# yumingj/C2-Matching

Hardware: AMD Instinct MI355X
Metric: LR-Ref image pairs/sec (160x160 LR, 500x500 Ref, 4x SR) (higher is better)
Workload: dtype f32

## Files before the change

### c2-matching_amd/c2m_amd/_lib.py

```python
import ctypes
import os

import torch

_HERE = os.path.dirname(os.path.abspath(__file__))
LIB_PATH = os.environ.get("C2M_LIB") or os.path.join(os.path.dirname(_HERE), "csrc", "libc2m_hip.so")
ABI_VERSION = 4

_vp, _i, _sz = ctypes.c_void_p, ctypes.c_int, ctypes.c_size_t
_lib = None


class ConvSrc(ctypes.Structure):
    _fields_ = [("ptr", _vp), ("C", _i), ("pix_pitch", _i), ("row_pitch", _i), ("img_pitch", ctypes.c_longlong)]


class Conv3x3Desc(ctypes.Structure):
    _fields_ = [("B", _i), ("H", _i), ("W", _i), ("Cin", _i), ("Cout", _i), ("nsrc", _i), ("src", ConvSrc * 2),
                ("wr", _vp), ("bias", _vp), ("act", _i), ("slope", ctypes.c_float), ("out_mode", _i), ("out", _vp),
                ("out_pix_pitch", _i), ("out_row_pitch", _i), ("out_img_pitch", ctypes.c_longlong), ("res1", _vp),
                ("res2", _vp), ("mask_out", _vp), ("flow", _vp), ("fh", _i), ("fw", _i), ("scale", _i), ("n_off", _i),
                ("abs_sum", _vp), ("algo", _i), ("cout_offset", _i), ("cout_total", _i),
                ("out2", _vp), ("out2_row_pitch", _i), ("out2_plane_pitch", ctypes.c_longlong),
                ("out2_img_pitch", ctypes.c_longlong), ("range_flag", _vp), ("io_flags", ctypes.c_int)]
# ... 8 lines not shown
    L.c2m_status_string.restype = ctypes.c_char_p
    L.c2m_status_string.argtypes = [_i]
    L.c2m_last_hip_error.restype = ctypes.c_char_p
    L.c2m_device_arch.argtypes = [ctypes.c_char_p, _i]
    L.c2m_profile_enable.argtypes = [_i]
    L.c2m_profile_collect.argtypes = [ctypes.POINTER(ctypes.c_float), ctypes.POINTER(_i), _i, ctypes.POINTER(_i)]
    L.c2m_feature_normalize_f32.argtypes = [_vp, _vp, _i, _i, _i, _vp]
    L.c2m_feature_match_workspace_bytes.restype = _sz
    L.c2m_feature_match_workspace_bytes.argtypes = [_i] * 5
    L.c2m_feature_match_workspace_bytes_c.restype = _sz
    L.c2m_feature_match_workspace_bytes_c.argtypes = [_i] * 6
    L.c2m_feature_match_skip_table.argtypes = [_i] * 5 + [ctypes.POINTER(ctypes.c_size_t), ctypes.POINTER(ctypes.c_int)]
    L.c2m_feature_match_index_f32.argtypes = [_vp, _vp, _vp] + [_i] * 12 + [_vp, _vp, _vp, _sz]
    L.c2m_feature_match_index_pre_f32.argtypes = [_vp, _vp, _vp] + [_i] * 12 + [_vp, _vp, _vp, _sz, _vp, _vp]
    L.c2m_feature_match_index_pre_f32.restype = _i
    L.c2m_feature_normalize_ss_f32.argtypes = [_vp, _vp, _i, _i, _i, _vp, _vp]
    L.c2m_feature_normalize_ss_f32.restype = _i
    L.c2m_feature_match_set_filter.argtypes = [_i]
    L.c2m_conv3x3_set_head_stores.argtypes = [_i]
    L.c2m_feature_match_filter_tables.argtypes = [_i] * 5 + [ctypes.POINTER(ctypes.c_size_t)] * 3 + [ctypes.POINTER(ctypes.c_int)]
    L.c2m_build_pre_offsets_f32.argtypes = [_vp, _vp, _i, _i, _i, _vp, _vp, _vp]
    for name in ("c2m_dcn_v2_forward_workspace_bytes",):
        getattr(L, name).restype = _sz
        getattr(L, name).argtypes = [_i] * 8
    L.c2m_dcn_v2_backward_workspace_bytes.restype = _sz
    L.c2m_dcn_v2_backward_workspace_bytes.argtypes = [_i] * 14
    L.c2m_dcn_v2_forward_f32.argtypes = [_vp] * 6 + [_i] * 14 + [_vp, _vp, _sz]
    L.c2m_dcn_v2_forward_bf16mma_f32.argtypes = [_vp] * 6 + [_i] * 14 + [_vp, _vp, _sz]
    L.c2m_dcn_v2_backward_f32.argtypes = [_vp] * 7 + [_i] * 14 + [_vp] * 5 + [_vp, _sz]
    L.c2m_dcn_fuse_offsets_f32.argtypes = [_vp, _vp, _vp, _i, _i, _i, _i, _i, _vp, _vp, _vp]
# ... 82 lines not shown
```

### c2-matching_amd/c2m_amd/ops.py

```python
import torch

from . import _lib


def _dev_f32(t, name):
    if not isinstance(t, torch.Tensor) or not t.is_cuda:
        raise _lib.C2MError(f"{name} must be a tensor on the GPU (the HIP path has no CPU fallback)")
    if t.dtype != torch.float32:
        raise _lib.C2MError(f"{name} must be float32, got {t.dtype}")
    return t if t.is_contiguous() else t.contiguous()


def _stream():
    return torch.cuda.current_stream().cuda_stream


def _pair(v):
    return (int(v), int(v)) if isinstance(v, int) else (int(v[0]), int(v[1]))


class NormalizedFeatures(torch.Tensor):

    @staticmethod
    def wrap(t, ss):
# ... 54 lines not shown
                                                         idx.data_ptr(), val.data_ptr(), ws.data_ptr(), nbytes,
                                                         ss_i.data_ptr() if ss_i is not None else None,
                                                         ss_r.data_ptr() if ss_r is not None else None),
                       "c2m_feature_match_index_pre_f32")
        mfma = (not force_generic) and p == 3 and si == 1 and sr == 1 and C in (64, 128, 256)
        if return_skip or _corr_diag.enabled:
            table = _skip_table(ws, (B, Hq, Wq, Hr, Wr)) if mfma else None
            if _corr_diag.enabled:
                _corr_diag.table = table
                _corr_diag.filter = _filter_tables(ws, (B, Hq, Wq, Hr, Wr), Hqp * Wqp) if mfma else None
            if return_skip:
                if table is None:
                    raise _lib.C2MError("return_skip: the duplicate-row table exists only on the MFMA kernel's path "
                                        "(patch 3, strides 1, C in 64/128/256, force_generic=False)")
                return idx, val, table
    return idx, val


class _CorrDiag:
    enabled = False
    table = None
    filter = None


_corr_diag = _CorrDiag()


class record_corr_skip_table:
    def __enter__(self):
        _corr_diag.enabled, _corr_diag.table = True, None
# ... 1181 lines not shown
```

### c2-matching_amd/csrc/corr_argmax.hip

```cpp
#include <stdlib.h>

#include "c2m_common.h"
#include "corr_filter.h"

namespace c2m {


__global__ void __launch_bounds__(256) feature_normalize_kernel(const float* __restrict__ x, int C, int HW,
                                                                 float* __restrict__ out, float* __restrict__ ss_out) {
  const int p = blockIdx.x * 256 + threadIdx.x;
  if (p >= HW) return;
  const float* xb = x + (size_t)blockIdx.y * C * HW + p;
  float* ob = out + (size_t)blockIdx.y * C * HW + p;
  float ss = 0.0f;
  for (int c = 0; c < C; ++c) {
    const float v = xb[(size_t)c * HW];
    ss = fmaf(v, v, ss);
  }
  const float nrm = sqrtf(ss);
  const float den = nrm > 1e-12f ? nrm : 1e-12f;
  float s2 = 0.0f;
  for (int c = 0; c < C; ++c) {
    const float o = xb[(size_t)c * HW] / den;
    ob[(size_t)c * HW] = o;
// ... 13 lines not shown
#pragma unroll
  for (int c = 0; c < C; ++c) v[c] = xb[(size_t)c * HW];
  float ss = 0.0f;
#pragma unroll
  for (int c = 0; c < C; ++c) ss = fmaf(v[c], v[c], ss);
  const float nrm = sqrtf(ss);
  const float den = nrm > 1e-12f ? nrm : 1e-12f;
  float s2 = 0.0f;
#pragma unroll
  for (int c = 0; c < C; ++c) {
    const float o = v[c] / den;
    ob[(size_t)c * HW] = o;
    s2 = fmaf(o, o, s2);
  }
  if (ss_out) ss_out[(size_t)blockIdx.y * HW + p] = s2;
}

__global__ void __launch_bounds__(256) pixel_sumsq_kernel(const float* __restrict__ x, int C, int HW,
                                                           float* __restrict__ ss) {
  const int p = blockIdx.x * 256 + threadIdx.x;
  if (p >= HW) return;
  const float* xb = x + (size_t)blockIdx.y * C * HW + p;
  float a = 0.0f;
  for (int c = 0; c < C; ++c) {
    const float v = xb[(size_t)c * HW];
    a = fmaf(v, v, a);
  }
  ss[(size_t)blockIdx.y * HW + p] = a;
}

// ... 392 lines not shown
    (void)hipMemsetAsync(row_eq, 0, sizeof(int) * (size_t)B * nxt * Hr, st);
  }
  hipLaunchKernelGGL(ref_row_run_kernel, dim3(ceil_div(B * nxt, 64)), dim3(64), 0, st, row_eq, Hr, B * nxt, skip);
  const int* need = nullptr;
  if (fws) {
    if (int rc = c2m::corrf::launch(st, fin, fref, B, C, Hq, Wq, Hr, Wr, inv, qden_buf, qden ? 1 : 0, skip, wsbase, *fws, max_idx,
                                    max_val))
      return rc;
    need = reinterpret_cast<const int*>(wsbase + fws->flags);
  }
  ProfileScope prof(C2M_KERNEL_CORR_MFMA, st);
  hipLaunchKernelGGL(kern, grid, dim3(NTHR), lds, st, fin, fref, Hq, Wq, Hr, Wr, tiles_y, tiles_x, inv ? inv : fin,
                     qden ? qden : fin, inv ? 1 : 0, qden ? 1 : 0, skip, need, max_idx, max_val);
  return check_launch();
}
}

namespace {
thread_local int g_filter_mode = -1;
}

extern "C" int c2m_feature_match_set_filter(int mode) {
  if (mode < -1 || mode > 1) return C2M_ERR_INVALID_ARG;
  g_filter_mode = mode;
  return C2M_OK;
}

extern "C" int c2m_feature_match_filter_tables(int B, int Hq, int Wq, int Hr, int Wr, size_t* cnt_offset, size_t* cand_offset,
                                               size_t* flags_offset, int* slots) {
  if (B <= 0 || Hq <= 0 || Wq <= 0 || Hr <= 0 || Wr <= 0 || !cnt_offset || !cand_offset || !flags_offset || !slots)
// ... 12 lines not shown
}

static int filter_channels(int C) { return (C == 64 || C == 128 || C == 256) ? C : 0; }

extern "C" size_t c2m_feature_match_workspace_bytes_c(int B, int C, int Hq, int Wq, int Hr, int Wr) {
  if (B <= 0 || C <= 0 || Hq <= 0 || Wq <= 0 || Hr <= 0 || Wr <= 0) return 0;
  return corr_ws(B, Hq, Wq, Hr, Wr, filter_channels(C)).total;
}

extern "C" int c2m_feature_match_skip_table(int B, int Hq, int Wq, int Hr, int Wr, size_t* byte_offset, int* x_tiles) {
  if (B <= 0 || Hq <= 0 || Wq <= 0 || Hr <= 0 || Wr <= 0 || !byte_offset || !x_tiles) return C2M_ERR_INVALID_ARG;
  const CorrWs ws = corr_ws(B, Hq, Wq, Hr, Wr);
  *byte_offset = ws.skip;
  *x_tiles = ws.nxt;
  return C2M_OK;
}

extern "C" int c2m_feature_match_index_f32(c2m_stream_t stream, const float* feat_in, const float* feat_ref, int B,
                                           int C, int Hq, int Wq, int Hr, int Wr, int patch, int in_stride,
                                           int ref_stride, int is_norm, int norm_input, int force_generic,
                                           int64_t* max_idx, float* max_val, void* workspace,
                                           size_t workspace_bytes) {
  return c2m_feature_match_index_pre_f32(stream, feat_in, feat_ref, B, C, Hq, Wq, Hr, Wr, patch, in_stride, ref_stride, is_norm,
                                         norm_input, force_generic, max_idx, max_val, workspace, workspace_bytes, nullptr, nullptr);
}

extern "C" int c2m_feature_match_index_pre_f32(c2m_stream_t stream, const float* feat_in, const float* feat_ref, int B,
                                               int C, int Hq, int Wq, int Hr, int Wr, int patch, int in_stride,
                                               int ref_stride, int is_norm, int norm_input, int force_generic,
                                               int64_t* max_idx, float* max_val, void* workspace,
// ... 11 lines not shown
  float* qden = reinterpret_cast<float*>(wsb + ws.qden);

  const int Hqp = (Hq - patch) / in_stride + 1, Wqp = (Wq - patch) / in_stride + 1;
  const int Hrp = (Hr - patch) / ref_stride + 1, Wrp = (Wr - patch) / ref_stride + 1;
  int rc;
  if (is_norm) {
    if (!ss_ref_pre)
      hipLaunchKernelGGL(pixel_sumsq_kernel, dim3(ceil_div(Hr * Wr, 256), B), dim3(256), 0, st, feat_ref, C, Hr * Wr,
                         ss_ref);
    hipLaunchKernelGGL(patch_norm_kernel, dim3(ceil_div(Hrp * Wrp, 256), B), dim3(256), 0, st, ss_ref_pre ? ss_ref_pre : ss_ref, Hr, Wr, patch,
                       ref_stride, Hrp, Wrp, 1, inv);
    if ((rc = check_launch()) != C2M_OK) return rc;
  }
  const bool fast = !force_generic && patch == 3 && in_stride == 1 && ref_stride == 1 &&
                    (C == 64 || C == 128 || C == 256);
  static const int filter_env = [] {
    const char* e = getenv("C2M_CORR_FILTER");
    return (e && e[0] == '0') ? 0 : 1;
  }();
  const int filter_on = g_filter_mode < 0 ? filter_env : g_filter_mode;
  const bool use_filter = fast && filter_on && is_norm && c2m::corrf::shapes_ok(B, C, Hq, Wq, Hr, Wr);
  if (norm_input || use_filter) {
    if (!ss_in_pre)
      hipLaunchKernelGGL(pixel_sumsq_kernel, dim3(ceil_div(Hq * Wq, 256), B), dim3(256), 0, st, feat_in, C, Hq * Wq,
                         ss_in);
    hipLaunchKernelGGL(patch_norm_kernel, dim3(ceil_div(Hqp * Wqp, 256), B), dim3(256), 0, st, ss_in_pre ? ss_in_pre : ss_in, Hq, Wq, patch,
                       in_stride, Hqp, Wqp, 0, qden);
    if ((rc = check_launch()) != C2M_OK) return rc;
  }
  const float* invp = is_norm ? inv : nullptr;
  const float* qdp = norm_input ? qden : nullptr;

  if (fast) {
    int* row_eq = reinterpret_cast<int*>(wsb + ws.row_eq);
    int2* skip = reinterpret_cast<int2*>(wsb + ws.skip);
    const c2m::corrf::Ws* fwsp = use_filter ? &ws.f : nullptr;
    static const int dedup = [] {
      const char* e = getenv("C2M_CORR_DEDUP");
      return (e && e[0] == '0') ? 0 : 1;
    }();
    if (C == 256)
      return launch_corr_mfma<256>(st, feat_in, feat_ref, B, Hq, Wq, Hr, Wr, invp, qdp, row_eq, skip, dedup, max_idx,
                                   max_val, fwsp, wsb, qden);
    if (C == 128)
      return launch_corr_mfma<128>(st, feat_in, feat_ref, B, Hq, Wq, Hr, Wr, invp, qdp, row_eq, skip, dedup, max_idx,
                                   max_val, fwsp, wsb, qden);
    return launch_corr_mfma<64>(st, feat_in, feat_ref, B, Hq, Wq, Hr, Wr, invp, qdp, row_eq, skip, dedup, max_idx,
                                max_val, fwsp, wsb, qden);
  }
  const size_t lds = sizeof(float) * (size_t)patch * patch * C;
  if (lds > 60 * 1024) return C2M_ERR_UNSUPPORTED;
  ProfileScope prof(C2M_KERNEL_CORR_GENERIC, st);
  hipLaunchKernelGGL(corr_argmax_generic_kernel, dim3(Hqp * Wqp, B), dim3(256), lds, st, feat_in, feat_ref, C, Hq, Wq,
                     Hr, Wr, patch, in_stride, ref_stride, Wqp, Hrp, Wrp, invp, qdp, max_idx, max_val);
  return check_launch();
// ... 17 lines not shown
```

### c2-matching_amd/csrc/corr_filter.h

```cpp
#pragma once
#include <hip/hip_runtime.h>
#include <stddef.h>
#include <stdint.h>

namespace c2m {
namespace corrf {

constexpr int WP = 28;
constexpr int KSLOT = 8;
constexpr int SCAN_ITEMS = 8192;
constexpr int CMAX = 256;

struct Ws {
  size_t qn, rn;
  size_t qpl;
  size_t rimg;
  size_t sb;
  size_t band;
  size_t eq;
  size_t cnt;
  size_t cand;
  size_t flags;
  size_t keys;
  size_t items;
// ... 27 lines not shown
  w.total = o;
  return w;
}

inline bool shapes_ok(int B, int C, int Hq, int Wq, int Hr, int Wr) {
  if (!(C == 64 || C == 128 || C == 256)) return false;
  if (Hr - 2 > 1024 || (Wr - 2 + WP - 1) / WP > 64) return false;
  const size_t lim = (size_t)1 << 31;
  const size_t nxt = (size_t)(Wr - 2 + WP - 1) / WP;
  return (size_t)Hq * Wq * C * 4 < lim && (size_t)Hr * Wr * C * 4 < lim && nxt * Hr * C * 128 < lim;
}

int launch(hipStream_t st, const float* fin, const float* fref, int B, int C, int Hq, int Wq, int Hr, int Wr, const float* inv,
           const float* qden, int norm_input, int2* skip, char* wsbase, const Ws& ws, int64_t* max_idx, float* max_val);

}
}
```

### c2-matching_amd/csrc/corr_filter.hip

```cpp
#include "corr_filter.h"

#include <stdlib.h>

#include "c2m_common.h"

namespace c2m {
namespace corrf {

constexpr int TQ = 16, TPQ = TQ - 2, WT = 32, NWAVE = 8, NTHR = NWAVE * 64, QPIX = TQ * TQ, SLAB = QPIX * WT, NIT = TPQ;
constexpr float BAND_ALPHA = 8.4e-5f, BAND_BETA = 1.0e-6f, INV_CAP = 2.0f;
constexpr float PIECE_SCALE = 16384.0f;
constexpr float SCORE_UNSCALE = 3.725290298461914e-9f;
constexpr float F16_MIN_NORMAL = 6.103515625e-5f;
constexpr int SCAN_FLAG = 0x40000000;
constexpr int SCAN_CAP = SCAN_ITEMS;
constexpr int SCAN_CHUNKS = 32, SCAN_STRIPES = 64;

typedef _Float16 f16x8 __attribute__((ext_vector_type(8)));


__global__ void __launch_bounds__(256) to_nhwc_kernel(const float* __restrict__ in, int C, int HW, float* __restrict__ out) {
  __shared__ float tile[64][65];
  const int b = blockIdx.z, c0 = blockIdx.y * 64, p0 = blockIdx.x * 64;
  const int tx = threadIdx.x & 63, ty = threadIdx.x >> 6;
// ... 48 lines not shown
  }
  if (bad) flags[0] = 1;
}

__device__ __forceinline__ void split2(float x, _Float16& h0, _Float16& h1, bool& bad) {
  const float xs = x * PIECE_SCALE;
  const float ax = __builtin_fabsf(xs);
  bad |= !(ax < 65520.0f);
  const _Float16 a = ax < F16_MIN_NORMAL ? (_Float16)0.0f : (_Float16)xs;
  const float r = xs - (float)a;
  const _Float16 c = __builtin_fabsf(r) < F16_MIN_NORMAL ? (_Float16)0.0f : (_Float16)r;
  h0 = a;
  h1 = c;
}

__device__ __forceinline__ void split8(const float* __restrict__ src, f16x8& p0, f16x8& p1, bool& bad) {
  const f32x4 a = *reinterpret_cast<const f32x4*>(src), c = *reinterpret_cast<const f32x4*>(src + 4);
#pragma unroll
  for (int e = 0; e < 4; ++e) {
    _Float16 h0, h1;
    split2(a[e], h0, h1, bad);
    p0[e] = h0; p1[e] = h1;
    split2(c[e], h0, h1, bad);
    p0[4 + e] = h0; p1[4 + e] = h1;
  }
}

__global__ void __launch_bounds__(256) split_query_kernel(const float* __restrict__ qn, int C, int HW, long long n8,
                                                           _Float16* __restrict__ qpl, int* __restrict__ flags) {
  const long long e = (long long)blockIdx.x * 256 + threadIdx.x;
  if (e >= n8) return;
  const int c8 = (int)(e % (C / 8));
  const long long gp = e / (C / 8);
  const long long b = gp / HW, p = gp - b * HW;
  f16x8 p0, p1;
  bool bad = false;
  split8(qn + (size_t)gp * C + c8 * 8, p0, p1, bad);
  _Float16* o = qpl + ((size_t)(b * 2) * HW + p) * C + c8 * 8;
  *reinterpret_cast<f16x8*>(o) = p0;
  *reinterpret_cast<f16x8*>(o + (size_t)HW * C) = p1;
// ... 32 lines not shown
    const u32x4 v = *me;
    if (x > 0) {
      const u32x4 o = *(me - C / 4);
      okl = v[0] == o[0] && v[1] == o[1] && v[2] == o[2] && v[3] == o[3];
    }
    if (y > 0) {
      const u32x4 o = *(me - (size_t)Wr * (C / 4));
      oku = v[0] == o[0] && v[1] == o[1] && v[2] == o[2] && v[3] == o[3];
    }
  }
  okl = __all(okl) && x > 0;
  oku = __all(oku) && y > 0;
  if (l == 0) {
    eq[gp] = okl ? 1 : 0;
    eq[npix + gp] = oku ? 1 : 0;
  }
}

__global__ void __launch_bounds__(256) cand_scale_kernel(const float* __restrict__ inv, const unsigned char* __restrict__ eq,
                                                          long long npix, int Hr, int Wr, int Hrp, int Wrp,
                                                          float* __restrict__ sc, int* __restrict__ flags, int* __restrict__ maxcol) {
  const int n0 = blockIdx.x * 256 + threadIdx.x, b = blockIdx.y;
  const bool in = n0 < Hrp * Wrp;
  const int n = in ? n0 : 0;
  const int ry = n / Wrp, rx = n - ry * Wrp;
  const unsigned char* el = eq + (size_t)b * Hr * Wr + (size_t)ry * Wr + rx;
  const unsigned char* eu = el + npix;
  bool dl = true, du = true;
#pragma unroll
  for (int i = 0; i < 3; ++i)
// ... 402 lines not shown
template <int C>
static int launch_filter_c(hipStream_t st, const _Float16* qpl, const _Float16* rimg, int B, int Hq, int Wq, int Hr, int Wr,
                           const float* sc, const float* band, const int2* skip, int* cnt, int* cand) {
  const int tiles_y = ceil_div(Hq - 2, TPQ), tiles_x = ceil_div(Wq - 2, TPQ);
  const size_t lds = sizeof(float) * (size_t)(3 * SLAB) + 2 * (size_t)C * 128;
  static const int pf = [] { const char* e = getenv("C2M_CORR_PF"); return (e && e[0] == '2') ? 2 : 1; }();
  static unsigned long long lds_set[2] = {0, 0};
  auto kern = pf == 1 ? &corr_filter_kernel<C, 1> : &corr_filter_kernel<C, 2>;
  if (int rc = ensure_dynamic_lds(reinterpret_cast<const void*>(kern), lds, lds_set[pf - 1])) return rc;
  ProfileScope prof(C2M_KERNEL_CORR_FILTER, st);
  hipLaunchKernelGGL(kern, dim3(B * tiles_y * tiles_x), dim3(NTHR), lds, st, qpl, rimg, Hq, Wq, Hr, Wr, tiles_y, tiles_x, sc, band,
                     skip, cnt, cand);
  return check_launch();
}

int launch(hipStream_t st, const float* fin, const float* fref, int B, int C, int Hq, int Wq, int Hr, int Wr, const float* inv,
           const float* qden, int norm_input, int2* skip, char* wsbase, const Ws& ws, int64_t* max_idx, float* max_val) {
  float* qn = reinterpret_cast<float*>(wsbase + ws.qn);
  float* rn = reinterpret_cast<float*>(wsbase + ws.rn);
  _Float16* qpl = reinterpret_cast<_Float16*>(wsbase + ws.qpl);
  _Float16* rimg = reinterpret_cast<_Float16*>(wsbase + ws.rimg);
  float* sc = reinterpret_cast<float*>(wsbase + ws.sb);
  float* band = reinterpret_cast<float*>(wsbase + ws.band);
  unsigned char* eq = reinterpret_cast<unsigned char*>(wsbase + ws.eq);
  int* cnt = reinterpret_cast<int*>(wsbase + ws.cnt);
  int* cand = reinterpret_cast<int*>(wsbase + ws.cand);
  int* flags = reinterpret_cast<int*>(wsbase + ws.flags);
  unsigned long long* keys = reinterpret_cast<unsigned long long*>(wsbase + ws.keys);
  ScanItem* items = reinterpret_cast<ScanItem*>(wsbase + ws.items);
  const int HWq = Hq * Wq, HWr = Hr * Wr, Hqp = Hq - 2, Wqp = Wq - 2, Hrp = Hr - 2, Wrp = Wr - 2;
  const int nxt = ceil_div(Wrp, WP);
  const long long nqp = (long long)B * Hqp * Wqp, npix_r = (long long)B * HWr;

  int* maxcol = reinterpret_cast<int*>(wsbase + ws.maxcol);
  static const int dead_tiles = [] { const char* e = getenv("C2M_CORR_DEAD_TILES"); return e ? atoi(e) : 1; }();
  (void)hipMemsetAsync(flags, 0, 32, st);
  (void)hipMemsetAsync(maxcol, 0, sizeof(int) * (size_t)B, st);
  hipLaunchKernelGGL(to_nhwc_split_kernel, dim3(ceil_div(HWq, 64), C / 64, B), dim3(256), 0, st, fin, C, HWq, qn, qpl, flags);
  hipLaunchKernelGGL(to_nhwc_kernel, dim3(ceil_div(HWr, 64), C / 64, B), dim3(256), 0, st, fref, C, HWr, rn);
  hipLaunchKernelGGL(split_ref_image_kernel, dim3(Hr, nxt, B), dim3(256), 0, st, rn, C, Hr, Wr, nxt, rimg, flags);
  hipLaunchKernelGGL(pixel_eq_kernel, dim3((unsigned)((npix_r + 3) / 4)), dim3(256), 0, st, rn, C, Hr, Wr, npix_r, eq);
  hipLaunchKernelGGL(cand_scale_kernel, dim3(ceil_div(Hrp * Wrp, 256), B), dim3(256), 0, st, inv, eq, npix_r, Hr, Wr, Hrp, Wrp, sc,
                     flags, maxcol);
  if (dead_tiles) hipLaunchKernelGGL(dead_tiles_kernel, dim3(ceil_div(B * nxt, 64)), dim3(64), 0, st, maxcol, nxt, B * nxt, Hr, skip);
  hipLaunchKernelGGL(band_kernel, dim3((unsigned)((nqp + 255) / 256)), dim3(256), 0, st, qden, nqp, band);
  int rc = check_launch();
  if (rc != C2M_OK) return rc;
  if (C == 256) rc = launch_filter_c<256>(st, qpl, rimg, B, Hq, Wq, Hr, Wr, sc, band, skip, cnt, cand);
  else if (C == 128) rc = launch_filter_c<128>(st, qpl, rimg, B, Hq, Wq, Hr, Wr, sc, band, skip, cnt, cand);
  else rc = launch_filter_c<64>(st, qpl, rimg, B, Hq, Wq, Hr, Wr, sc, band, skip, cnt, cand);
  if (rc != C2M_OK) return rc;
  {
    ProfileScope prof(C2M_KERNEL_CORR_RESOLVE, st);
    hipLaunchKernelGGL(corr_resolve_kernel, dim3((unsigned)((nqp + 27) / 28)), dim3(256), 0, st, qn, rn, C, Hq, Wq, Hr, Wr, inv, qden,
                       norm_input, cnt, cand, nqp, keys, items, flags, max_idx, max_val);
    hipLaunchKernelGGL(corr_scan_kernel, dim3(SCAN_CHUNKS, SCAN_STRIPES), dim3(256), 0, st, qn, rn, C, Hq, Wq, Hr, Wr, inv, items, flags,
                       keys);
    hipLaunchKernelGGL(corr_scan_finish_kernel, dim3(8), dim3(256), 0, st, items, flags, keys, qden, norm_input, max_idx, max_val);
  }
  return check_launch();
}

}
}
```

### c2-matching_amd/mmsr/models/archs/corres_generation_arch.py

```python
import logging

import torch
import torch.nn as nn

from c2m_amd import ops as _ops
from mmsr.models.archs.vgg_arch import VGGFeatureExtractor

logger = logging.getLogger('base')


class PreOffsets(dict):

    _SCALE = {'relu3_1': 1, 'relu2_1': 2, 'relu1_1': 4}

    def __init__(self, max_idx, h=None, w=None):
        super().__init__()
        if isinstance(max_idx, torch.Tensor):
            dict.__setitem__(self, 'max_idx', max_idx)
        else:
            for k, v in dict(max_idx).items():
                dict.__setitem__(self, k, v)
            if not dict.__contains__(self, 'max_idx'):
                raise TypeError("PreOffsets needs the arg-max index map (a tensor, or a mapping with key 'max_idx')")
        mi = dict.__getitem__(self, 'max_idx')
# ... 34 lines not shown
        super(CorrespondenceGenerationArch, self).__init__()
        self.patch_size = patch_size
        self.stride = stride
        self.vgg_layer_list = vgg_layer_list
        self.vgg = VGGFeatureExtractor(layer_name_list=vgg_layer_list, vgg_type=vgg_type)
        self.vgg.grouped8_taps = ('relu1_1',)
        self.vgg.fast_conv = True

    def index_to_flow(self, max_idx):
        h, w = max_idx.shape
        (flow,) = _ops.build_pre_offsets(max_idx[None].contiguous(), h + 2, w + 2, scales=(1,))
        return flow[:, 0]

    @torch.no_grad()
    def match(self, dense_features):
        feat_in = _ops.feature_normalize(dense_features['dense_features1'].float(), with_sumsq=True)
        feat_ref = _ops.feature_normalize(dense_features['dense_features2'].float(), with_sumsq=True)
        return _ops.feature_match_index_batched(feat_in, feat_ref, self.patch_size, self.stride, self.stride,
                                                is_norm=True, norm_input=True)

    def forward(self, dense_features, img_ref_hr):
        if self.patch_size != 3 or self.stride != 1:
            raise NotImplementedError('pre-offset generation is defined for patch_size=3, stride=1')
        h, w = dense_features['dense_features1'].shape[2:]
        max_idx, _ = self.match(dense_features)
        pre_offset = PreOffsets(max_idx, h, w)
        img_ref_feat = self.vgg(img_ref_hr)
        return pre_offset, img_ref_feat
```

### include/c2m_hip.h

```cpp
#ifndef C2M_HIP_H
#define C2M_HIP_H

#include <stddef.h>
#include <stdint.h>

#ifdef __cplusplus
extern "C" {
#endif

typedef void* c2m_stream_t;

typedef enum c2m_status {
  C2M_OK = 0,
  C2M_ERR_INVALID_ARG = 1,
  C2M_ERR_UNSUPPORTED = 2,
  C2M_ERR_WORKSPACE = 3,
  C2M_ERR_LAUNCH = 4,
  C2M_ERR_NO_DEVICE = 5
} c2m_status;

int c2m_abi_version(void);
const char* c2m_status_string(int status);
const char* c2m_last_hip_error(void);
int c2m_device_arch(char* buf, int buflen);
// ... 20 lines not shown
int c2m_feature_match_set_filter(int mode);

int c2m_conv3x3_set_head_stores(int mode);

int c2m_feature_match_filter_tables(int B, int Hq, int Wq, int Hr, int Wr, size_t* cnt_offset, size_t* cand_offset,
                                    size_t* flags_offset, int* slots);

int c2m_feature_match_index_f32(c2m_stream_t stream, const float* feat_in, const float* feat_ref, int B, int C,
                                int Hq, int Wq, int Hr, int Wr, int patch, int in_stride, int ref_stride,
                                int is_norm, int norm_input, int force_generic, int64_t* max_idx, float* max_val,
                                void* workspace, size_t workspace_bytes);
int c2m_feature_match_index_pre_f32(c2m_stream_t stream, const float* feat_in, const float* feat_ref, int B, int C,
                                    int Hq, int Wq, int Hr, int Wr, int patch, int in_stride, int ref_stride,
                                    int is_norm, int norm_input, int force_generic, int64_t* max_idx, float* max_val,
                                    void* workspace, size_t workspace_bytes, const float* ss_in_pre, const float* ss_ref_pre);

int c2m_build_pre_offsets_f32(c2m_stream_t stream, const int64_t* max_idx, int B, int h, int w, float* off3,
                              float* off2, float* off1);

size_t c2m_dcn_v2_forward_workspace_bytes(int B, int C, int H, int W, int Co, int kh, int kw, int dg);
int c2m_dcn_v2_forward_f32(c2m_stream_t stream, const float* input, const float* weight, const float* bias,
                           const float* offset, const float* mask, int B, int C, int H, int W, int Co, int kh, int kw,
                           int sh, int sw, int ph, int pw, int dh, int dw, int dg, float* output, void* workspace,
                           size_t workspace_bytes);

int c2m_dcn_v2_forward_bf16mma_f32(c2m_stream_t stream, const float* input, const float* weight, const float* bias,
                                   const float* offset, const float* mask, int B, int C, int H, int W, int Co, int kh,
                                   int kw, int sh, int sw, int ph, int pw, int dh, int dw, int dg, float* output,
                                   void* workspace, size_t workspace_bytes);

// ... 120 lines not shown
```

Measured before the change: 119.9.

## Fuse feature normalization into correlation filter prep from raw features

Adds a raw-input entry point for the correlation-argmax path. Instead of normalizing features to NCHW and then transposing them to NHWC for the filter, one kernel normalizes, writes NHWC, and emits the fp16 split planes. A single kernel also builds the split ref image and the row/pixel equality tables. The NCHW normalized tensors are only produced, via conditional kernels, when the filter flags a fallback to the MFMA kernel. This cuts several passes over feature memory and launches, but it adds a new code path, an extra scratch allocation per call, and 256-float register arrays per thread.

```diff
diff --git a/c2-matching_amd/c2m_amd/_lib.py b/c2-matching_amd/c2m_amd/_lib.py
--- a/c2-matching_amd/c2m_amd/_lib.py
+++ b/c2-matching_amd/c2m_amd/_lib.py
@@ -46,6 +46,8 @@
     L.c2m_feature_match_index_f32.argtypes = [_vp, _vp, _vp] + [_i] * 12 + [_vp, _vp, _vp, _sz]
     L.c2m_feature_match_index_pre_f32.argtypes = [_vp, _vp, _vp] + [_i] * 12 + [_vp, _vp, _vp, _sz, _vp, _vp]
     L.c2m_feature_match_index_pre_f32.restype = _i
+    L.c2m_feature_match_index_raw_f32.argtypes = [_vp, _vp, _vp] + [_i] * 12 + [_vp, _vp, _vp, _sz, _vp, _vp]
+    L.c2m_feature_match_index_raw_f32.restype = _i
     L.c2m_feature_normalize_ss_f32.argtypes = [_vp, _vp, _i, _i, _i, _vp, _vp]
     L.c2m_feature_normalize_ss_f32.restype = _i
     L.c2m_feature_match_set_filter.argtypes = [_i]
diff --git a/c2-matching_amd/c2m_amd/ops.py b/c2-matching_amd/c2m_amd/ops.py
--- a/c2-matching_amd/c2m_amd/ops.py
+++ b/c2-matching_amd/c2m_amd/ops.py
@@ -92,6 +92,37 @@
                     raise _lib.C2MError("return_skip: the duplicate-row table exists only on the MFMA kernel's path "
                                         "(patch 3, strides 1, C in 64/128/256, force_generic=False)")
                 return idx, val, table
+    return idx, val
+
+
+def feature_match_index_raw(raw_in, raw_ref, patch_size=3, stride=1, norm_input=True):
+    ok = all(isinstance(t, torch.Tensor) and t.is_cuda and t.dtype == torch.float32 and t.dim() == 4 for t in (raw_in, raw_ref))
+    if not ok or raw_in.shape[:2] != raw_ref.shape[:2] or raw_in.device != raw_ref.device:
+        return None
+    fi, fr = raw_in.contiguous(), raw_ref.contiguous()
+    B, C, Hq, Wq = fi.shape
+    Hr, Wr = fr.shape[2:]
+    p, s = int(patch_size), int(stride)
+    if min(Hq, Wq, Hr, Wr) < p or p != 3 or s != 1 or C not in (64, 128, 256):
+        return None
+    Hqp, Wqp = (Hq - p) // s + 1, (Wq - p) // s + 1
+    L = _lib.lib()
+    with torch.cuda.device(fi.device):
+        nbytes = L.c2m_feature_match_workspace_bytes_c(B, C, Hq, Wq, Hr, Wr)
+        ws = torch.empty(nbytes, dtype=torch.uint8, device=fi.device)
+        idx = torch.empty((B, Hqp, Wqp), dtype=torch.int64, device=fi.device)
+        val = torch.empty((B, Hqp, Wqp), dtype=torch.float32, device=fi.device)
+        ni, nr = torch.empty_like(fi), torch.empty_like(fr)
+        with _apply_switch("filter"):
+            rc = L.c2m_feature_match_index_raw_f32(_stream(), fi.data_ptr(), fr.data_ptr(), B, C, Hq, Wq, Hr, Wr, p, s, s, 1,
+                                                   int(bool(norm_input)), 0, idx.data_ptr(), val.data_ptr(), ws.data_ptr(), nbytes,
+                                                   ni.data_ptr(), nr.data_ptr())
+        if rc == 2:
+            return None
+        _lib.check(rc, "c2m_feature_match_index_raw_f32")
+        if _corr_diag.enabled:
+            _corr_diag.table = _skip_table(ws, (B, Hq, Wq, Hr, Wr))
+            _corr_diag.filter = _filter_tables(ws, (B, Hq, Wq, Hr, Wr), Hqp * Wqp)
     return idx, val
 
 
diff --git a/c2-matching_amd/csrc/corr_argmax.hip b/c2-matching_amd/csrc/corr_argmax.hip
--- a/c2-matching_amd/csrc/corr_argmax.hip
+++ b/c2-matching_amd/csrc/corr_argmax.hip
@@ -51,6 +51,26 @@
     s2 = fmaf(o, o, s2);
   }
   if (ss_out) ss_out[(size_t)blockIdx.y * HW + p] = s2;
+}
+
+template <int C>
+__global__ void __launch_bounds__(256, 1) feature_normalize_if_kernel(const float* __restrict__ x, int HW, float* __restrict__ out,
+                                                                       const int* __restrict__ need) {
+  if (*need == 0) return;
+  const int p = blockIdx.x * 256 + threadIdx.x;
+  if (p >= HW) return;
+  const float* xb = x + (size_t)blockIdx.y * C * HW + p;
+  float* ob = out + (size_t)blockIdx.y * C * HW + p;
+  float v[C];
+#pragma unroll
+  for (int c = 0; c < C; ++c) v[c] = xb[(size_t)c * HW];
+  float ss = 0.0f;
+#pragma unroll
+  for (int c = 0; c < C; ++c) ss = fmaf(v[c], v[c], ss);
+  const float nrm = sqrtf(ss);
+  const float den = nrm > 1e-12f ? nrm : 1e-12f;
+#pragma unroll
+  for (int c = 0; c < C; ++c) ob[(size_t)c * HW] = v[c] / den;
 }
 
 __global__ void __launch_bounds__(256) pixel_sumsq_kernel(const float* __restrict__ x, int C, int HW,
@@ -473,6 +493,34 @@
                      qden ? qden : fin, inv ? 1 : 0, qden ? 1 : 0, skip, need, max_idx, max_val);
   return check_launch();
 }
+
+template <int C>
+int launch_corr_raw(hipStream_t st, const float* raw_in, const float* raw_ref, int B, int Hq, int Wq, int Hr, int Wr, float* ss_in,
+                    float* ss_ref, float* inv, float* qden, int norm_input, int* row_eq, int2* skip, int dedup, int64_t* max_idx,
+                    float* max_val, const c2m::corrf::Ws& fws, char* wsbase, float* norm_in, float* norm_ref) {
+  using namespace c2m::corr;
+  const int tiles_y = ceil_div(Hq - 2, TPQ), tiles_x = ceil_div(Wq - 2, TPQ);
+  const int Hqp = Hq - 2, Wqp = Wq - 2, Hrp = Hr - 2, Wrp = Wr - 2, nxt = ceil_div(Wrp, WP);
+  const size_t lds = sizeof(float) * (size_t)(3 * SLAB + 2 * C * WT);
+  static unsigned long long lds_set[2] = {0, 0};
+  const bool dma16 = (Wr % 4 == 0) && (reinterpret_cast<uintptr_t>(norm_ref) % 16 == 0);
+  auto kern = dma16 ? &corr_argmax_mfma_kernel<C, true> : &corr_argmax_mfma_kernel<C, false>;
+  if (int rc = ensure_dynamic_lds(reinterpret_cast<const void*>(kern), lds, lds_set[dma16])) return rc;
+  if (int rc = c2m::corrf::prepare_raw(st, raw_in, raw_ref, B, C, Hq, Wq, Hr, Wr, ss_in, ss_ref, row_eq, wsbase, fws)) return rc;
+  if (!dedup) (void)hipMemsetAsync(row_eq, 0, sizeof(int) * (size_t)B * nxt * Hr, st);
+  hipLaunchKernelGGL(patch_norm_kernel, dim3(ceil_div(Hrp * Wrp, 256), B), dim3(256), 0, st, ss_ref, Hr, Wr, 3, 1, Hrp, Wrp, 1, inv);
+  hipLaunchKernelGGL(patch_norm_kernel, dim3(ceil_div(Hqp * Wqp, 256), B), dim3(256), 0, st, ss_in, Hq, Wq, 3, 1, Hqp, Wqp, 0, qden);
+  hipLaunchKernelGGL(ref_row_run_kernel, dim3(ceil_div(B * nxt, 64)), dim3(64), 0, st, row_eq, Hr, B * nxt, skip);
+  if (int rc = check_launch()) return rc;
+  if (int rc = c2m::corrf::sweep(st, B, C, Hq, Wq, Hr, Wr, inv, qden, norm_input, skip, wsbase, fws, max_idx, max_val)) return rc;
+  const int* need = reinterpret_cast<const int*>(wsbase + fws.flags);
+  hipLaunchKernelGGL(feature_normalize_if_kernel<C>, dim3(ceil_div(Hq * Wq, 256), B), dim3(256), 0, st, raw_in, Hq * Wq, norm_in, need);
+  hipLaunchKernelGGL(feature_normalize_if_kernel<C>, dim3(ceil_div(Hr * Wr, 256), B), dim3(256), 0, st, raw_ref, Hr * Wr, norm_ref, need);
+  ProfileScope prof(C2M_KERNEL_CORR_MFMA, st);
+  hipLaunchKernelGGL(kern, dim3(B * tiles_y * tiles_x), dim3(NTHR), lds, st, norm_in, norm_ref, Hq, Wq, Hr, Wr, tiles_y, tiles_x, inv,
+                     norm_input ? qden : norm_in, 1, norm_input ? 1 : 0, skip, need, max_idx, max_val);
+  return check_launch();
+}
 }
 
 namespace {
@@ -515,6 +563,53 @@
   *byte_offset = ws.skip;
   *x_tiles = ws.nxt;
   return C2M_OK;
+}
+
+static int filter_enabled() {
+  static const int filter_env = [] {
+    const char* e = getenv("C2M_CORR_FILTER");
+    return (e && e[0] == '0') ? 0 : 1;
+  }();
+  return g_filter_mode < 0 ? filter_env : g_filter_mode;
+}
+
+static int dedup_enabled() {
+  static const int dedup = [] {
+    const char* e = getenv("C2M_CORR_DEDUP");
+    return (e && e[0] == '0') ? 0 : 1;
+  }();
+  return dedup;
+}
+
+extern "C" int c2m_feature_match_index_raw_f32(c2m_stream_t stream, const float* feat_in_raw, const float* feat_ref_raw, int B, int C,
+                                               int Hq, int Wq, int Hr, int Wr, int patch, int in_stride, int ref_stride, int is_norm,
+                                               int norm_input, int force_generic, int64_t* max_idx, float* max_val, void* workspace,
+                                               size_t workspace_bytes, float* norm_in_scratch, float* norm_ref_scratch) {
+  if (!feat_in_raw || !feat_ref_raw || !max_idx || !max_val || !norm_in_scratch || !norm_ref_scratch) return C2M_ERR_INVALID_ARG;
+  if (B <= 0 || C <= 0 || patch <= 0 || in_stride <= 0 || ref_stride <= 0) return C2M_ERR_INVALID_ARG;
+  if (Hq < patch || Wq < patch || Hr < patch || Wr < patch) return C2M_ERR_INVALID_ARG;
+  if (force_generic || patch != 3 || in_stride != 1 || ref_stride != 1 || !is_norm || !filter_enabled() ||
+      !c2m::corrf::shapes_ok(B, C, Hq, Wq, Hr, Wr))
+    return C2M_ERR_UNSUPPORTED;
+  const CorrWs ws = corr_ws(B, Hq, Wq, Hr, Wr, filter_channels(C));
+  if (!workspace || workspace_bytes < ws.total) return C2M_ERR_WORKSPACE;
+  hipStream_t st = as_stream(stream);
+  char* wsb = static_cast<char*>(workspace);
+  float* ss_ref = reinterpret_cast<float*>(wsb + ws.ss_ref);
+  float* inv = reinterpret_cast<float*>(wsb + ws.inv);
+  float* ss_in = reinterpret_cast<float*>(wsb + ws.ss_in);
+  float* qden = reinterpret_cast<float*>(wsb + ws.qden);
+  int* row_eq = reinterpret_cast<int*>(wsb + ws.row_eq);
+  int2* skip = reinterpret_cast<int2*>(wsb + ws.skip);
+  const int ni = norm_input ? 1 : 0, dd = dedup_enabled();
+  if (C == 256)
+    return launch_corr_raw<256>(st, feat_in_raw, feat_ref_raw, B, Hq, Wq, Hr, Wr, ss_in, ss_ref, inv, qden, ni, row_eq, skip, dd, max_idx,
+                                max_val, ws.f, wsb, norm_in_scratch, norm_ref_scratch);
+  if (C == 128)
+    return launch_corr_raw<128>(st, feat_in_raw, feat_ref_raw, B, Hq, Wq, Hr, Wr, ss_in, ss_ref, inv, qden, ni, row_eq, skip, dd, max_idx,
+                                max_val, ws.f, wsb, norm_in_scratch, norm_ref_scratch);
+  return launch_corr_raw<64>(st, feat_in_raw, feat_ref_raw, B, Hq, Wq, Hr, Wr, ss_in, ss_ref, inv, qden, ni, row_eq, skip, dd, max_idx,
+                             max_val, ws.f, wsb, norm_in_scratch, norm_ref_scratch);
 }
 
 extern "C" int c2m_feature_match_index_f32(c2m_stream_t stream, const float* feat_in, const float* feat_ref, int B,
@@ -556,11 +651,7 @@
   }
   const bool fast = !force_generic && patch == 3 && in_stride == 1 && ref_stride == 1 &&
                     (C == 64 || C == 128 || C == 256);
-  static const int filter_env = [] {
-    const char* e = getenv("C2M_CORR_FILTER");
-    return (e && e[0] == '0') ? 0 : 1;
-  }();
-  const int filter_on = g_filter_mode < 0 ? filter_env : g_filter_mode;
+  const int filter_on = filter_enabled();
   const bool use_filter = fast && filter_on && is_norm && c2m::corrf::shapes_ok(B, C, Hq, Wq, Hr, Wr);
   if (norm_input || use_filter) {
     if (!ss_in_pre)
@@ -577,10 +668,7 @@
     int* row_eq = reinterpret_cast<int*>(wsb + ws.row_eq);
     int2* skip = reinterpret_cast<int2*>(wsb + ws.skip);
     const c2m::corrf::Ws* fwsp = use_filter ? &ws.f : nullptr;
-    static const int dedup = [] {
-      const char* e = getenv("C2M_CORR_DEDUP");
-      return (e && e[0] == '0') ? 0 : 1;
-    }();
+    const int dedup = dedup_enabled();
     if (C == 256)
       return launch_corr_mfma<256>(st, feat_in, feat_ref, B, Hq, Wq, Hr, Wr, invp, qdp, row_eq, skip, dedup, max_idx,
                                    max_val, fwsp, wsb, qden);
diff --git a/c2-matching_amd/csrc/corr_filter.h b/c2-matching_amd/csrc/corr_filter.h
--- a/c2-matching_amd/csrc/corr_filter.h
+++ b/c2-matching_amd/csrc/corr_filter.h
@@ -65,5 +65,10 @@
 int launch(hipStream_t st, const float* fin, const float* fref, int B, int C, int Hq, int Wq, int Hr, int Wr, const float* inv,
            const float* qden, int norm_input, int2* skip, char* wsbase, const Ws& ws, int64_t* max_idx, float* max_val);
 
+int prepare_raw(hipStream_t st, const float* fin_raw, const float* fref_raw, int B, int C, int Hq, int Wq, int Hr, int Wr, float* ss_in,
+                float* ss_ref, int* row_eq, char* wsbase, const Ws& ws);
+int sweep(hipStream_t st, int B, int C, int Hq, int Wq, int Hr, int Wr, const float* inv, const float* qden, int norm_input, int2* skip,
+          char* wsbase, const Ws& ws, int64_t* max_idx, float* max_val);
+
 }
 }
diff --git a/c2-matching_amd/csrc/corr_filter.hip b/c2-matching_amd/csrc/corr_filter.hip
--- a/c2-matching_amd/csrc/corr_filter.hip
+++ b/c2-matching_amd/csrc/corr_filter.hip
@@ -86,8 +86,7 @@
   h1 = c;
 }
 
-__device__ __forceinline__ void split8(const float* __restrict__ src, f16x8& p0, f16x8& p1, bool& bad) {
-  const f32x4 a = *reinterpret_cast<const f32x4*>(src), c = *reinterpret_cast<const f32x4*>(src + 4);
+__device__ __forceinline__ void split8(f32x4 a, f32x4 c, f16x8& p0, f16x8& p1, bool& bad) {
 #pragma unroll
   for (int e = 0; e < 4; ++e) {
     _Float16 h0, h1;
@@ -96,6 +95,10 @@
     split2(c[e], h0, h1, bad);
     p0[4 + e] = h0; p1[4 + e] = h1;
   }
+}
+
+__device__ __forceinline__ void split8(const float* __restrict__ src, f16x8& p0, f16x8& p1, bool& bad) {
+  split8(*reinterpret_cast<const f32x4*>(src), *reinterpret_cast<const f32x4*>(src + 4), p0, p1, bad);
 }
 
 __global__ void __launch_bounds__(256) split_query_kernel(const float* __restrict__ qn, int C, int HW, long long n8,
@@ -158,6 +161,120 @@
   if (l == 0) {
     eq[gp] = okl ? 1 : 0;
     eq[npix + gp] = oku ? 1 : 0;
+  }
+}
+
+
+template <int C, bool SPLIT>
+__global__ void __launch_bounds__(256, 1) normalize_nhwc_kernel(const float* __restrict__ x, int HW, float* __restrict__ out,
+                                                                 float* __restrict__ ss_out, _Float16* __restrict__ qpl,
+                                                                 int* __restrict__ flags) {
+  __shared__ __attribute__((aligned(16))) float tile[4][64 * 64];
+  const int b = blockIdx.y, l = threadIdx.x & 63, w = threadIdx.x >> 6;
+  const int p0 = blockIdx.x * 256 + w * 64, p = p0 + l;
+  const float* xb = x + (size_t)b * C * HW + min(p, HW - 1);
+  float v[C];
+#pragma unroll
+  for (int c = 0; c < C; ++c) v[c] = xb[(size_t)c * HW];
+  float ss = 0.0f;
+#pragma unroll
+  for (int c = 0; c < C; ++c) ss = fmaf(v[c], v[c], ss);
+  const float nrm = sqrtf(ss);
+  const float den = nrm > 1e-12f ? nrm : 1e-12f;
+  float s2 = 0.0f;
+#pragma unroll
+  for (int c = 0; c < C; ++c) {
+    v[c] = v[c] / den;
+    s2 = fmaf(v[c], v[c], s2);
+  }
+  if (p < HW) ss_out[(size_t)blockIdx.y * HW + p] = s2;
+
+  float* tw = tile[w];
+  const int pl = l >> 4, g = l & 15;
+  typedef _Float16 f16x4 __attribute__((ext_vector_type(4)));
+  bool bad = false;
+#pragma unroll
+  for (int k = 0; k < C / 64; ++k) {
+#pragma unroll
+    for (int gg = 0; gg < 16; ++gg) {
+      f32x4 o;
+#pragma unroll
+      for (int e = 0; e < 4; ++e) o[e] = v[64 * k + 4 * gg + e];
+      *reinterpret_cast<f32x4*>(tw + l * 64 + ((gg ^ (l & 15)) * 4)) = o;
+    }
+    __syncthreads();
+#pragma unroll
+    for (int i = 0; i < 16; ++i) {
+      const int px = 4 * i + pl, pp = p0 + px;
+      const f32x4 o = *reinterpret_cast<const f32x4*>(tw + px * 64 + ((g ^ (px & 15)) * 4));
+      if (pp < HW) {
+        const size_t at = ((size_t)b * HW + pp) * C + 64 * k + 4 * g;
+        *reinterpret_cast<f32x4*>(out + at) = o;
+        if constexpr (SPLIT) {
+          f16x4 q0, q1;
+#pragma unroll
+          for (int e = 0; e < 4; ++e) {
+            _Float16 h0, h1;
+            split2(o[e], h0, h1, bad);
+            q0[e] = h0; q1[e] = h1;
+          }
+          _Float16* q = qpl + at + (size_t)b * HW * C;
+          *reinterpret_cast<f16x4*>(q) = q0;
+          *reinterpret_cast<f16x4*>(q + (size_t)HW * C) = q1;
+        }
+      }
+    }
+    __syncthreads();
+  }
+  if (SPLIT && bad) flags[0] = 1;
+}
+
+__global__ void __launch_bounds__(256) ref_image_eq_kernel(const float* __restrict__ rn, int C, int Hr, int Wr, int nxt,
+                                                            _Float16* __restrict__ rimg, unsigned char* __restrict__ eq, long long npix,
+                                                            int* __restrict__ row_eq, int* __restrict__ flags) {
+  __shared__ int ndl[32], ndu[32];
+  const int y = blockIdx.x, xt = blockIdx.y, b = blockIdx.z;
+  if (threadIdx.x < 32) { ndl[threadIdx.x] = 0; ndu[threadIdx.x] = 0; }
+  __syncthreads();
+  _Float16* img = rimg + (((size_t)b * nxt + xt) * Hr + y) * ((size_t)C * 64);
+  const size_t plane = (size_t)(C / 16) * 512;
+  typedef unsigned u32x4 __attribute__((ext_vector_type(4)));
+  const int j = threadIdx.x & 31, x = xt * WP + j;
+  bool bad = false, dl = false, du = false;
+  for (int u = threadIdx.x; u < C * 4; u += 256) {
+    const int kh = (u >> 5) & 1, t = u >> 6;
+    f16x8 p0 = {0, 0, 0, 0, 0, 0, 0, 0}, p1 = p0;
+    if (x < Wr) {
+      const u32x4* src = reinterpret_cast<const u32x4*>(rn + (((size_t)b * Hr + y) * Wr + x) * C + 16 * t + 8 * kh);
+      const u32x4 a = src[0], c = src[1];
+      split8(__builtin_bit_cast(f32x4, a), __builtin_bit_cast(f32x4, c), p0, p1, bad);
+      if (x > 0) {
+        const u32x4 d = (a ^ src[-(C / 4)]) | (c ^ src[1 - C / 4]);
+        dl |= (d[0] | d[1] | d[2] | d[3]) != 0u;
+      }
+      if (y > 0) {
+        const u32x4* up = src - (size_t)Wr * (C / 4);
+        const u32x4 d = (a ^ up[0]) | (c ^ up[1]);
+        du |= (d[0] | d[1] | d[2] | d[3]) != 0u;
+      }
+    }
+    _Float16* o = img + (size_t)(t * 2 + kh) * 256 + j * 8;
+    *reinterpret_cast<f16x8*>(o) = p0;
+    *reinterpret_cast<f16x8*>(o + plane) = p1;
+  }
+  if (dl) ndl[j] = 1;
+  if (du) ndu[j] = 1;
+  if (bad) flags[0] = 1;
+  __syncthreads();
+  if (threadIdx.x < 64) {
+    const bool live = threadIdx.x < 32 && x < Wr;
+    if (live && (j < WP || xt == nxt - 1)) {
+      const size_t gp = ((size_t)b * Hr + y) * Wr + x;
+      eq[gp] = (x > 0 && !ndl[j]) ? 1 : 0;
+      eq[npix + gp] = (y > 0 && !ndu[j]) ? 1 : 0;
+    }
+    const bool differs = __any(live && ndu[j] != 0);
+    if (threadIdx.x == 0 && y > 0) row_eq[((size_t)b * nxt + xt) * Hr + y - 1] = differs ? 0 : 1;
   }
 }
 
@@ -590,52 +707,94 @@
   return check_launch();
 }
 
-int launch(hipStream_t st, const float* fin, const float* fref, int B, int C, int Hq, int Wq, int Hr, int Wr, const float* inv,
-           const float* qden, int norm_input, int2* skip, char* wsbase, const Ws& ws, int64_t* max_idx, float* max_val) {
-  float* qn = reinterpret_cast<float*>(wsbase + ws.qn);
-  float* rn = reinterpret_cast<float*>(wsbase + ws.rn);
-  _Float16* qpl = reinterpret_cast<_Float16*>(wsbase + ws.qpl);
-  _Float16* rimg = reinterpret_cast<_Float16*>(wsbase + ws.rimg);
-  float* sc = reinterpret_cast<float*>(wsbase + ws.sb);
-  float* band = reinterpret_cast<float*>(wsbase + ws.band);
-  unsigned char* eq = reinterpret_cast<unsigned char*>(wsbase + ws.eq);
-  int* cnt = reinterpret_cast<int*>(wsbase + ws.cnt);
-  int* cand = reinterpret_cast<int*>(wsbase + ws.cand);
-  int* flags = reinterpret_cast<int*>(wsbase + ws.flags);
-  unsigned long long* keys = reinterpret_cast<unsigned long long*>(wsbase + ws.keys);
-  ScanItem* items = reinterpret_cast<ScanItem*>(wsbase + ws.items);
-  const int HWq = Hq * Wq, HWr = Hr * Wr, Hqp = Hq - 2, Wqp = Wq - 2, Hrp = Hr - 2, Wrp = Wr - 2;
+namespace {
+struct Bufs {
+  float *qn, *rn, *sc, *band;
+  _Float16 *qpl, *rimg;
+  unsigned char* eq;
+  int *cnt, *cand, *flags, *maxcol;
+  unsigned long long* keys;
+  ScanItem* items;
+  Bufs(char* wsbase, const Ws& ws)
+      : qn(reinterpret_cast<float*>(wsbase + ws.qn)), rn(reinterpret_cast<float*>(wsbase + ws.rn)),
+        sc(reinterpret_cast<float*>(wsbase + ws.sb)), band(reinterpret_cast<float*>(wsbase + ws.band)),
+        qpl(reinterpret_cast<_Float16*>(wsbase + ws.qpl)), rimg(reinterpret_cast<_Float16*>(wsbase + ws.rimg)),
+        eq(reinterpret_cast<unsigned char*>(wsbase + ws.eq)), cnt(reinterpret_cast<int*>(wsbase + ws.cnt)),
+        cand(reinterpret_cast<int*>(wsbase + ws.cand)), flags(reinterpret_cast<int*>(wsbase + ws.flags)),
+        maxcol(reinterpret_cast<int*>(wsbase + ws.maxcol)), keys(reinterpret_cast<unsigned long long*>(wsbase + ws.keys)),
+        items(reinterpret_cast<ScanItem*>(wsbase + ws.items)) {}
+};
+}
+
+static int prepare(hipStream_t st, const float* fin, const float* fref, int B, int C, int Hq, int Wq, int Hr, int Wr, const Bufs& w) {
+  const int HWq = Hq * Wq, HWr = Hr * Wr, nxt = ceil_div(Wr - 2, WP);
+  const long long npix_r = (long long)B * HWr;
+  (void)hipMemsetAsync(w.flags, 0, 32, st);
+  (void)hipMemsetAsync(w.maxcol, 0, sizeof(int) * (size_t)B, st);
+  hipLaunchKernelGGL(to_nhwc_split_kernel, dim3(ceil_div(HWq, 64), C / 64, B), dim3(256), 0, st, fin, C, HWq, w.qn, w.qpl, w.flags);
+  hipLaunchKernelGGL(to_nhwc_kernel, dim3(ceil_div(HWr, 64), C / 64, B), dim3(256), 0, st, fref, C, HWr, w.rn);
+  hipLaunchKernelGGL(split_ref_image_kernel, dim3(Hr, nxt, B), dim3(256), 0, st, w.rn, C, Hr, Wr, nxt, w.rimg, w.flags);
+  hipLaunchKernelGGL(pixel_eq_kernel, dim3((unsigned)((npix_r + 3) / 4)), dim3(256), 0, st, w.rn, C, Hr, Wr, npix_r, w.eq);
+  return check_launch();
+}
+
+template <int C>
+static void launch_prepare_raw_c(hipStream_t st, const float* fin_raw, const float* fref_raw, int B, int HWq, int HWr, float* ss_in,
+                                 float* ss_ref, const Bufs& w) {
+  hipLaunchKernelGGL((normalize_nhwc_kernel<C, true>), dim3(ceil_div(HWq, 256), B), dim3(256), 0, st, fin_raw, HWq, w.qn, ss_in, w.qpl,
+                     w.flags);
+  hipLaunchKernelGGL((normalize_nhwc_kernel<C, false>), dim3(ceil_div(HWr, 256), B), dim3(256), 0, st, fref_raw, HWr, w.rn, ss_ref,
+                     (_Float16*)nullptr, w.flags);
+}
+
+int prepare_raw(hipStream_t st, const float* fin_raw, const float* fref_raw, int B, int C, int Hq, int Wq, int Hr, int Wr, float* ss_in,
+                float* ss_ref, int* row_eq, char* wsbase, const Ws& ws) {
+  const Bufs w(wsbase, ws);
+  const int HWq = Hq * Wq, HWr = Hr * Wr, nxt = ceil_div(Wr - 2, WP);
+  (void)hipMemsetAsync(w.flags, 0, 32, st);
+  (void)hipMemsetAsync(w.maxcol, 0, sizeof(int) * (size_t)B, st);
+  if (C == 256) launch_prepare_raw_c<256>(st, fin_raw, fref_raw, B, HWq, HWr, ss_in, ss_ref, w);
+  else if (C == 128) launch_prepare_raw_c<128>(st, fin_raw, fref_raw, B, HWq, HWr, ss_in, ss_ref, w);
+  else if (C == 64) launch_prepare_raw_c<64>(st, fin_raw, fref_raw, B, HWq, HWr, ss_in, ss_ref, w);
+  else return C2M_ERR_UNSUPPORTED;
+  hipLaunchKernelGGL(ref_image_eq_kernel, dim3(Hr, nxt, B), dim3(256), 0, st, w.rn, C, Hr, Wr, nxt, w.rimg, w.eq, (long long)B * HWr,
+                     row_eq, w.flags);
+  return check_launch();
+}
+
+int sweep(hipStream_t st, int B, int C, int Hq, int Wq, int Hr, int Wr, const float* inv, const float* qden, int norm_input, int2* skip,
+          char* wsbase, const Ws& ws, int64_t* max_idx, float* max_val) {
+  const Bufs w(wsbase, ws);
+  const int Hqp = Hq - 2, Wqp = Wq - 2, Hrp = Hr - 2, Wrp = Wr - 2;
   const int nxt = ceil_div(Wrp, WP);
-  const long long nqp = (long long)B * Hqp * Wqp, npix_r = (long long)B * HWr;
-
-  int* maxcol = reinterpret_cast<int*>(wsbase + ws.maxcol);
+  const long long nqp = (long long)B * Hqp * Wqp, npix_r = (long long)B * Hr * Wr;
   static const int dead_tiles = [] { const char* e = getenv("C2M_CORR_DEAD_TILES"); return e ? atoi(e) : 1; }();
-  (void)hipMemsetAsync(flags, 0, 32, st);
-  (void)hipMemsetAsync(maxcol, 0, sizeof(int) * (size_t)B, st);
-  hipLaunchKernelGGL(to_nhwc_split_kernel, dim3(ceil_div(HWq, 64), C / 64, B), dim3(256), 0, st, fin, C, HWq, qn, qpl, flags);
-  hipLaunchKernelGGL(to_nhwc_kernel, dim3(ceil_div(HWr, 64), C / 64, B), dim3(256), 0, st, fref, C, HWr, rn);
-  hipLaunchKernelGGL(split_ref_image_kernel, dim3(Hr, nxt, B), dim3(256), 0, st, rn, C, Hr, Wr, nxt, rimg, flags);
-  hipLaunchKernelGGL(pixel_eq_kernel, dim3((unsigned)((npix_r + 3) / 4)), dim3(256), 0, st, rn, C, Hr, Wr, npix_r, eq);
-  hipLaunchKernelGGL(cand_scale_kernel, dim3(ceil_div(Hrp * Wrp, 256), B), dim3(256), 0, st, inv, eq, npix_r, Hr, Wr, Hrp, Wrp, sc,
-                     flags, maxcol);
-  if (dead_tiles) hipLaunchKernelGGL(dead_tiles_kernel, dim3(ceil_div(B * nxt, 64)), dim3(64), 0, st, maxcol, nxt, B * nxt, Hr, skip);
-  hipLaunchKernelGGL(band_kernel, dim3((unsigned)((nqp + 255) / 256)), dim3(256), 0, st, qden, nqp, band);
+  hipLaunchKernelGGL(cand_scale_kernel, dim3(ceil_div(Hrp * Wrp, 256), B), dim3(256), 0, st, inv, w.eq, npix_r, Hr, Wr, Hrp, Wrp, w.sc,
+                     w.flags, w.maxcol);
+  if (dead_tiles) hipLaunchKernelGGL(dead_tiles_kernel, dim3(ceil_div(B * nxt, 64)), dim3(64), 0, st, w.maxcol, nxt, B * nxt, Hr, skip);
+  hipLaunchKernelGGL(band_kernel, dim3((unsigned)((nqp + 255) / 256)), dim3(256), 0, st, qden, nqp, w.band);
   int rc = check_launch();
   if (rc != C2M_OK) return rc;
-  if (C == 256) rc = launch_filter_c<256>(st, qpl, rimg, B, Hq, Wq, Hr, Wr, sc, band, skip, cnt, cand);
-  else if (C == 128) rc = launch_filter_c<128>(st, qpl, rimg, B, Hq, Wq, Hr, Wr, sc, band, skip, cnt, cand);
-  else rc = launch_filter_c<64>(st, qpl, rimg, B, Hq, Wq, Hr, Wr, sc, band, skip, cnt, cand);
+  if (C == 256) rc = launch_filter_c<256>(st, w.qpl, w.rimg, B, Hq, Wq, Hr, Wr, w.sc, w.band, skip, w.cnt, w.cand);
+  else if (C == 128) rc = launch_filter_c<128>(st, w.qpl, w.rimg, B, Hq, Wq, Hr, Wr, w.sc, w.band, skip, w.cnt, w.cand);
+  else rc = launch_filter_c<64>(st, w.qpl, w.rimg, B, Hq, Wq, Hr, Wr, w.sc, w.band, skip, w.cnt, w.cand);
   if (rc != C2M_OK) return rc;
   {
     ProfileScope prof(C2M_KERNEL_CORR_RESOLVE, st);
-    hipLaunchKernelGGL(corr_resolve_kernel, dim3((unsigned)((nqp + 27) / 28)), dim3(256), 0, st, qn, rn, C, Hq, Wq, Hr, Wr, inv, qden,
-                       norm_input, cnt, cand, nqp, keys, items, flags, max_idx, max_val);
-    hipLaunchKernelGGL(corr_scan_kernel, dim3(SCAN_CHUNKS, SCAN_STRIPES), dim3(256), 0, st, qn, rn, C, Hq, Wq, Hr, Wr, inv, items, flags,
-                       keys);
-    hipLaunchKernelGGL(corr_scan_finish_kernel, dim3(8), dim3(256), 0, st, items, flags, keys, qden, norm_input, max_idx, max_val);
+    hipLaunchKernelGGL(corr_resolve_kernel, dim3((unsigned)((nqp + 27) / 28)), dim3(256), 0, st, w.qn, w.rn, C, Hq, Wq, Hr, Wr, inv, qden,
+                       norm_input, w.cnt, w.cand, nqp, w.keys, w.items, w.flags, max_idx, max_val);
+    hipLaunchKernelGGL(corr_scan_kernel, dim3(SCAN_CHUNKS, SCAN_STRIPES), dim3(256), 0, st, w.qn, w.rn, C, Hq, Wq, Hr, Wr, inv, w.items,
+                       w.flags, w.keys);
+    hipLaunchKernelGGL(corr_scan_finish_kernel, dim3(8), dim3(256), 0, st, w.items, w.flags, w.keys, qden, norm_input, max_idx, max_val);
   }
   return check_launch();
 }
 
-}
-}
+int launch(hipStream_t st, const float* fin, const float* fref, int B, int C, int Hq, int Wq, int Hr, int Wr, const float* inv,
+           const float* qden, int norm_input, int2* skip, char* wsbase, const Ws& ws, int64_t* max_idx, float* max_val) {
+  if (int rc = prepare(st, fin, fref, B, C, Hq, Wq, Hr, Wr, Bufs(wsbase, ws))) return rc;
+  return sweep(st, B, C, Hq, Wq, Hr, Wr, inv, qden, norm_input, skip, wsbase, ws, max_idx, max_val);
+}
+
+}
+}
diff --git a/c2-matching_amd/mmsr/models/archs/corres_generation_arch.py b/c2-matching_amd/mmsr/models/archs/corres_generation_arch.py
--- a/c2-matching_amd/mmsr/models/archs/corres_generation_arch.py
+++ b/c2-matching_amd/mmsr/models/archs/corres_generation_arch.py
@@ -72,8 +72,12 @@
 
     @torch.no_grad()
     def match(self, dense_features):
-        feat_in = _ops.feature_normalize(dense_features['dense_features1'].float(), with_sumsq=True)
-        feat_ref = _ops.feature_normalize(dense_features['dense_features2'].float(), with_sumsq=True)
+        raw_in, raw_ref = dense_features['dense_features1'].float(), dense_features['dense_features2'].float()
+        fused = _ops.feature_match_index_raw(raw_in, raw_ref, self.patch_size, self.stride, norm_input=True)
+        if fused is not None:
+            return fused
+        feat_in = _ops.feature_normalize(raw_in, with_sumsq=True)
+        feat_ref = _ops.feature_normalize(raw_ref, with_sumsq=True)
         return _ops.feature_match_index_batched(feat_in, feat_ref, self.patch_size, self.stride, self.stride,
                                                 is_norm=True, norm_input=True)
 
diff --git a/include/c2m_hip.h b/include/c2m_hip.h
--- a/include/c2m_hip.h
+++ b/include/c2m_hip.h
@@ -58,6 +58,10 @@
                                     int Hq, int Wq, int Hr, int Wr, int patch, int in_stride, int ref_stride,
                                     int is_norm, int norm_input, int force_generic, int64_t* max_idx, float* max_val,
                                     void* workspace, size_t workspace_bytes, const float* ss_in_pre, const float* ss_ref_pre);
+int c2m_feature_match_index_raw_f32(c2m_stream_t stream, const float* feat_in_raw, const float* feat_ref_raw, int B, int C,
+                                    int Hq, int Wq, int Hr, int Wr, int patch, int in_stride, int ref_stride,
+                                    int is_norm, int norm_input, int force_generic, int64_t* max_idx, float* max_val,
+                                    void* workspace, size_t workspace_bytes, float* norm_in_scratch, float* norm_ref_scratch);
 
 int c2m_build_pre_offsets_f32(c2m_stream_t stream, const int64_t* max_idx, int B, int h, int w, float* off3,
                               float* off2, float* off1);
```

Result: no change. 120.4, median of 6 (+0.4%).
